# facebookresearch/CODD

Measured on AMD Instinct MI355X. Metric: frames/sec full CODD forward @960x540 (whole job), higher is better.
Workload: dtype f32 (split-bf16 MFMA operands, f32 accumulate; HITNet + context network + Fusion exact f32); 1 GPU; full CODD (HITNetMF + Motion/RAFT3D iters=16 + Fusion) 960x540 padded to 960x576, max_disp=320, one video per GPU, steady-state frames (idx>=1), synthetic stereo sequence, random-init weights; conv_precision=split, hip_graph=True, frames_per_gpu=304, prewarm_frames=150, side_streams=True, library=codd_amd/csrc/libcodd_hip.so, full=False

## Files before the change

### codd_amd/csrc/conv.hip

```cpp
#include "conv_quad_kernel.h"
#include <stdio.h>
#include <stdlib.h>

CONV_ALL_GROUPS(CONV_DECLARE)
CONVQ_ALL(CONVQ_DECLARE)
CONVQ_MULTI(CONVQM_DECLARE)


__global__ void conv_pack_kernel(const float* __restrict__ w, float* __restrict__ wp, int Cout, int Cin, int ntaps,
                                 int mb, int ck, int wrow, int nchunks, long long total, long long co_stride,
                                 long long ci_stride, float scale) {
  long long e = (long long)blockIdx.x * blockDim.x + threadIdx.x;
  if (e >= total) return;
  int col = (int)(e % wrow);
  long long t = e / wrow;
  int c = (int)(t % ck); t /= ck;
  int tap = (int)(t % ntaps); t /= ntaps;
  int chunk = (int)(t % nchunks);
  int cog = (int)(t / nchunks);
  int co = cog * 16 * mb + col, ci = chunk * ck + c;
  float v = 0.f;
  if (col < 16 * mb && co < Cout && ci < Cin) v = w[(size_t)co * co_stride + (size_t)ci * ci_stride + tap] * scale;
  wp[e] = v;
}

__global__ void conv_pack_quad_kernel(const float* __restrict__ w, float* __restrict__ wp, int Cout, int Cin, int ntaps,
                                      int mb, int ck, int nchunks, long long total) {
  long long e = (long long)blockIdx.x * blockDim.x + threadIdx.x;
  if (e >= total) return;
  const int q = (int)(e & 3);
  long long t = e >> 2;
  const int col = (int)(t % (16 * mb)); t /= 16 * mb;
  const int cq = (int)(t % (ck >> 2)); t /= ck >> 2;
  const int tap = (int)(t % ntaps); t /= ntaps;
  const int chunk = (int)(t % nchunks);
  const int cog = (int)(t / nchunks);
  const int co = cog * 16 * mb + col, ci = chunk * ck + 4 * cq + q;
  wp[e] = (co < Cout && ci < Cin) ? w[((size_t)co * Cin + ci) * ntaps + tap] : 0.f;
}

extern "C" long long codd_conv2d_packed_size_quad(int Cout, int Cin, int kh, int kw, int mb, int ck) {
  if (mb < 1 || !(ck == 16 || ck == 32)) return -1;
  return (long long)cdiv(Cout, 16 * mb) * cdiv(Cin, ck) * (kh * kw) * ck * 16 * mb;
}

extern "C" int codd_conv2d_pack_weights_quad(const float* w, float* wpacked, int Cout, int Cin, int kh, int kw, int mb,
                                             int ck, void* stream) {
  const long long total = codd_conv2d_packed_size_quad(Cout, Cin, kh, kw, mb, ck);
  if (total <= 0 || !w || !wpacked) return CODD_EINVAL;
  conv_pack_quad_kernel<<<cdiv(total, 256), 256, 0, (hipStream_t)stream>>>(w, wpacked, Cout, Cin, kh * kw, mb, ck,
                                                                           cdiv(Cin, ck), total);
  CODD_LAUNCH_CHECK();
  return CODD_OK;
}

static inline int wrow_of(int mb) { return 16 * mb + ((mb & 1) ? 0 : 16); }

extern "C" long long codd_conv2d_packed_size(int Cout, int Cin, int kh, int kw, int mb, int ck) {
  if (mb < 1 || ck < 4 || (ck & 3)) return -1;
  long long ncog = cdiv(Cout, 16 * mb), nchunks = cdiv(Cin, ck);
  return ncog * nchunks * (long long)(kh * kw) * ck * wrow_of(mb);
}

extern "C" int codd_conv2d_pack_weights_ex(const float* w, float* wpacked, int Cout, int Cin, int kh, int kw, int mb,
                                           int ck, long long co_stride, long long ci_stride, float scale,
                                           void* stream) {
  long long total = codd_conv2d_packed_size(Cout, Cin, kh, kw, mb, ck);
  if (total <= 0 || !w || !wpacked) return CODD_EINVAL;
  int nchunks = cdiv(Cin, ck);
  conv_pack_kernel<<<cdiv(total, 256), 256, 0, (hipStream_t)stream>>>(w, wpacked, Cout, Cin, kh * kw, mb, ck,
                                                                      wrow_of(mb), nchunks, total, co_stride,
                                                                      ci_stride, scale);
  CODD_LAUNCH_CHECK();
  return CODD_OK;
}

extern "C" int codd_conv2d_pack_weights(const float* w, float* wpacked, int Cout, int Cin, int kh, int kw, int mb,
                                        int ck, void* stream) {
  return codd_conv2d_pack_weights_ex(w, wpacked, Cout, Cin, kh, kw, mb, ck, (long long)Cin * kh * kw,
                                     (long long)kh * kw, 1.f, stream);
}

template <int NW, int NPB, int MB, int WREG, int IREG>
static int launch_conv(const ConvK& k, size_t lds, int grid, hipStream_t s) {
  if (lds > 64 * 1024) {
    hipError_t e = hipFuncSetAttribute((const void*)conv_mfma_kernel<NW, NPB, MB, WREG, IREG>,
                                       hipFuncAttributeMaxDynamicSharedMemorySize, (int)lds);
    if (e != hipSuccess) return (int)e;
  }
  conv_mfma_kernel<NW, NPB, MB, WREG, IREG><<<grid, NW * 64, lds, s>>>(k);
  CODD_LAUNCH_CHECK();
  return CODD_OK;
}

template <int NPB, int MB>
static int launch_conv_regs(const ConvK& k, size_t lds, int grid, hipStream_t s) {
  const int wr = cdiv(k.wchunk >> 2, 256), ir = cdiv(k.nunits, 256);
  if (wr <= 4 && ir <= 4) return launch_conv<4, NPB, MB, 4, 4>(k, lds, grid, s);
  if (wr <= 4 && ir <= 8) return launch_conv<4, NPB, MB, 4, 8>(k, lds, grid, s);
  if (wr <= 12 && ir <= 4) return launch_conv<4, NPB, MB, 12, 4>(k, lds, grid, s);
  if (wr <= 12 && ir <= 8) return launch_conv<4, NPB, MB, 12, 8>(k, lds, grid, s);
  if (wr <= 16 && ir <= 8) return launch_conv<4, NPB, MB, 16, 8>(k, lds, grid, s);
  return CODD_EUNSUPPORTED;
}

template <int NW, int MB>
static int launch_conv_nwx(const ConvK& k, size_t lds, int grid, hipStream_t s) {
  const int wr = cdiv(k.wchunk >> 2, NW * 64), ir = cdiv(k.nunits, NW * 64);
  if (wr <= 8 && ir <= 4) return launch_conv<NW, 1, MB, 8, 4>(k, lds, grid, s);
  if (wr <= 16 && ir <= 4) return launch_conv<NW, 1, MB, 16, 4>(k, lds, grid, s);
  return CODD_EUNSUPPORTED;
}

template <int NW, int NPB, int MB, int WREG, int QREG>
static int launch_quad(const ConvK& k, size_t lds, int grid, hipStream_t s) {
  if (lds > 64 * 1024) {
    hipError_t e = hipFuncSetAttribute((const void*)conv_quad_kernel<NW, NPB, MB, WREG, QREG>,
                                       hipFuncAttributeMaxDynamicSharedMemorySize, (int)lds);
    if (e != hipSuccess) return (int)e;
  }
  conv_quad_kernel<NW, NPB, MB, WREG, QREG><<<grid, NW * 64, lds, s>>>(k);
  CODD_LAUNCH_CHECK();
  return CODD_OK;
}

static int launch_quad_any(const ConvK& k, int nw, size_t lds, int grid, hipStream_t s) {
  const codd_conv_params& p = k.p;
  const int nt = nw * 64, wr = cdiv(k.wchunk >> 2, nt), qr = cdiv((p.ck >> 2) * k.upc, nt);
#define Q(W, N, M, R, QQ) if (nw == W && p.npb == N && p.mb == M && wr <= R && qr <= QQ) return launch_quad<W, N, M, R, QQ>(k, lds, grid, s);
  Q(4, 1, 1, 8, 2) Q(4, 1, 2, 8, 1) Q(4, 1, 2, 16, 2) Q(4, 1, 4, 12, 1) Q(4, 1, 4, 16, 2)
  Q(4, 2, 1, 8, 2) Q(4, 2, 2, 8, 2) Q(4, 2, 2, 16, 2) Q(4, 2, 4, 12, 2) Q(4, 2, 4, 16, 2)
  Q(4, 4, 1, 8, 4) Q(4, 4, 2, 8, 4)
  Q(9, 1, 1, 8, 1) Q(9, 1, 2, 8, 1) Q(9, 1, 4, 8, 1) Q(9, 1, 4, 16, 1)
#undef Q
  return CODD_EUNSUPPORTED;
}

int codd_conv2d_bf16(const codd_conv_params* pp, void* stream, int dry_run);

extern "C" int codd_conv2d_check(const codd_conv_params* pp) {
  if (!pp || pp->layout != 2) return CODD_EINVAL;
  return codd_conv2d_bf16(pp, nullptr, 1);
}

static int conv_fill(const codd_conv_params* pp, ConvK& k, size_t& lds, long long& grid, int& nw) {
  k.p = *pp;
  const codd_conv_params& p = k.p;
  if (!p.in0.ptr || !p.out || !p.wpacked || p.C0 <= 0 || p.C1 < 0 || (p.C1 > 0 && !p.in1.ptr)) return CODD_EINVAL;
  if (p.ck < 4 || (p.ck & 3) || p.B < 1 || p.Cout < 1 || p.kh < 1 || p.kw < 1 || p.pad_l < 0 || p.pad_t < 0)
    return CODD_EINVAL;
  if (!(p.mb == 1 || p.mb == 2 || p.mb == 4) || !(p.npb == 1 || p.npb == 2 || p.npb == 4)) return CODD_EINVAL;
  if (p.store_mode && (p.kh != 1 || p.kw != 1 || p.res1.ptr || p.res2.ptr || p.post.ptr)) return CODD_EUNSUPPORTED;
  k.cin = p.C0 + p.C1;
  k.nchunks = cdiv(k.cin, p.ck);
  k.ntaps = p.kh * p.kw;
  const int xb = p.npb >= 2 ? 2 : 1, rpw = p.npb / xb;
  nw = p.nw ? p.nw : 4;
  if (nw != 4 && (!(nw == 9 || nw == 2 || nw == 8) || p.npb != 1)) return CODD_EUNSUPPORTED;
  k.th = nw * rpw;
  k.tw = 16 * xb;
  k.thi = (k.th - 1) * p.sy + (p.kh - 1) * p.dil_y + 1;
  k.twi = (k.tw - 1) * p.sx + (p.kw - 1) * p.dil_x + 1;
  k.xoff = (4 - (p.pad_l % 4)) % 4;
  k.twp = ((k.xoff + k.twi + 3) / 4) * 4;
  k.twp4 = k.twp / 4;
  k.upc = k.thi * k.twp4;
  k.nunits = p.ck * k.upc;
  const int per = k.thi * k.twp;
  if (p.sx == 1) k.chs = ((per + 15) / 32) * 32 + 16;
  else k.chs = per + 4;
  k.wrow = wrow_of(p.mb);
  k.wchunk = k.ntaps * p.ck * k.wrow;
  k.tiles_x = cdiv(p.Wout, k.tw);
  k.tiles_y = cdiv(p.Hout, k.th);
  k.cout_eff = p.store_mode ? 4 * p.Cout : p.Cout;
  k.ncog = cdiv(k.cout_eff, 16 * p.mb);
  const size_t hwb = (size_t)p.Hin * p.Win * sizeof(float);
  k.vec_ok = (p.Win % 4 == 0) && ((uintptr_t)p.in0.ptr % 16 == 0) && (hwb % 16 == 0) &&
             (p.C1 == 0 || (uintptr_t)p.in1.ptr % 16 == 0);
  lds = ((size_t)k.wchunk + (size_t)p.ck * k.chs) * sizeof(float);
  if (p.layout == 1) {
    if (!(p.ck == 16 || p.ck == 32) || p.sx > 2 || !k.vec_ok) return CODD_EUNSUPPORTED;
    k.wchunk = k.ntaps * p.ck * 16 * p.mb;
    lds = ((size_t)k.wchunk + (size_t)p.ck * k.thi * k.twp) * sizeof(float);
  } else if (p.layout != 0) {
    return CODD_EINVAL;
  }
  if (lds > 160 * 1024) return CODD_EUNSUPPORTED;
  grid = (long long)k.tiles_x * k.tiles_y * k.ncog * p.B;
  if (grid <= 0 || grid > 0x7fffffffLL) return CODD_EINVAL;
  k.xcd = 1;
  return CODD_OK;
}

extern "C" int codd_conv2d(const codd_conv_params* pp, void* stream) {
  if (!pp) return CODD_EINVAL;
  if (pp->layout != 2 && (pp->dil2 || pp->gate)) return CODD_EUNSUPPORTED;
  if (pp->layout == 2) {
    const codd_conv_params& q = *pp;
    if (!q.xs || (!q.out && !q.xso) || !q.wpacked || q.C0 <= 0 || q.C1 < 0 || q.B < 1 || q.Cout < 1 || q.kh < 1 || q.kw < 1 ||
        q.pad_l < 0 || q.pad_t < 0)
      return CODD_EINVAL;
    if (q.store_mode && (q.kh != 1 || q.kw != 1 || q.res1.ptr || q.res2.ptr || q.post.ptr)) return CODD_EUNSUPPORTED;
    return codd_conv2d_bf16(pp, stream, 0);
  }
  ConvK k;
  size_t lds;
  long long grid;
  int nw;
  const int rc = conv_fill(pp, k, lds, grid, nw);
  if (rc != CODD_OK) return rc;
  const codd_conv_params& p = k.p;
  hipStream_t s = (hipStream_t)stream;
  if (p.layout == 1) return launch_quad_any(k, nw, lds, (int)grid, s);
#define CASEW(W, M) if (nw == W && p.mb == M) return launch_conv_nwx<W, M>(k, lds, (int)grid, s)
  CASEW(9, 1); CASEW(9, 2); CASEW(9, 4); CASEW(2, 1); CASEW(2, 2); CASEW(2, 4); CASEW(8, 1); CASEW(8, 2); CASEW(8, 4);
#undef CASEW
#define CASE(N, M) if (p.npb == N && p.mb == M) return launch_conv_regs<N, M>(k, lds, (int)grid, s)
  CASE(1, 1); CASE(1, 2); CASE(1, 4);
  CASE(2, 1); CASE(2, 2); CASE(2, 4);
  CASE(4, 1); CASE(4, 2); CASE(4, 4);
#undef CASE
  return CODD_EUNSUPPORTED;
}

template <int NW, int NPB, int MB, int WREG, int QREG>
static int launch_quad_multi(const ConvKN& kn, size_t lds, int grid, hipStream_t s) {
  if (lds > 64 * 1024) {
    hipError_t e = hipFuncSetAttribute((const void*)conv_quad_multi_kernel<NW, NPB, MB, WREG, QREG>,
                                       hipFuncAttributeMaxDynamicSharedMemorySize, (int)lds);
    if (e != hipSuccess) return (int)e;
  }
  conv_quad_multi_kernel<NW, NPB, MB, WREG, QREG><<<grid, NW * 64, lds, s>>>(kn);
  CODD_LAUNCH_CHECK();
  return CODD_OK;
}

extern "C" int codd_conv2d_multi(const codd_conv_params* ps, int n, void* stream) {
  if (!ps || n < 1 || n > CONVQ_MULTI_MAX) return CODD_EINVAL;
  if (n == 1) return codd_conv2d(ps, stream);
  ConvKN kn;
  memset(&kn, 0, sizeof(kn));
  size_t lds = 0;
  long long total = 0;
  int wr = 0, qr = 0;
  for (int i = 0; i < n; ++i) {
    size_t l;
    long long g;
    int nw;
    if (ps[i].layout != 1) return CODD_EUNSUPPORTED;
    const int rc = conv_fill(&ps[i], kn.k[i], l, g, nw);
    if (rc != CODD_OK) return rc;
    const codd_conv_params& p = kn.k[i].p;
    if (nw != 4 || p.npb != 1 || p.mb != ps[0].mb || !(p.mb == 1 || p.mb == 2)) return CODD_EUNSUPPORTED;
    const int w_ = cdiv(kn.k[i].wchunk >> 2, 256), q_ = cdiv((p.ck >> 2) * kn.k[i].upc, 256);
    wr = w_ > wr ? w_ : wr;
    qr = q_ > qr ? q_ : qr;
    lds = l > lds ? l : lds;
    kn.start[i] = (int)total;
    total += g;
  }
  for (int i = n; i <= CONVQ_MULTI_MAX; ++i) kn.start[i] = (int)total;
  if (total > 0x7fffffffLL) return CODD_EINVAL;
  hipStream_t s = (hipStream_t)stream;
  if (ps[0].mb == 1 && wr <= 8 && qr <= 2) return launch_quad_multi<4, 1, 1, 8, 2>(kn, lds, (int)total, s);
  if (ps[0].mb == 2 && wr <= 16 && qr <= 2) return launch_quad_multi<4, 1, 2, 16, 2>(kn, lds, (int)total, s);
  return CODD_EUNSUPPORTED;
}

extern "C" int codd_avgpool2(const float* in, int BC, int h, int w, float* out, void* stream);

#define CORR_MB 4
#define CORR_CK 32
extern "C" long long codd_allpairs_corr_scratch(int B, int D, int h, int w) {
  long long packed = codd_conv2d_packed_size(h * w, D, 1, 1, CORR_MB, CORR_CK);
  long long pooled = 0;
  int hh = h, ww = w;
  for (int i = 1; i < 4; ++i) { hh >>= 1; ww >>= 1; pooled += (long long)D * hh * ww; }
  return (long long)B * (packed + pooled);
}

extern "C" int codd_allpairs_corr(const float* f1, const float* f2, int B, int D, int h, int w, float* lvl0,
                                  float* lvl1, float* lvl2, float* lvl3, float* scratch, void* stream) {
  if (!f1 || !f2 || !lvl0 || !lvl1 || !lvl2 || !lvl3 || !scratch || (h >> 3) < 1 || (w >> 3) < 1) return CODD_EINVAL;
  const int N = h * w;
  const long long packed = codd_conv2d_packed_size(N, D, 1, 1, CORR_MB, CORR_CK);
  float* lv[4] = {lvl0, lvl1, lvl2, lvl3};
  for (int b = 0; b < B; ++b) {
    float* wp = scratch + (size_t)b * packed;
    int rc = codd_conv2d_pack_weights_ex(f1 + (size_t)b * D * N, wp, N, D, 1, 1, CORR_MB, CORR_CK, 1, N, 1.f / 16.f,
                                         stream);
    if (rc) return rc;
  }
  float* pool = scratch + (size_t)B * packed;
  const float* src = f2;
  int hh = h, ww = w;
  for (int i = 0; i < 4; ++i) {
    if (i > 0) {
      int rc = codd_avgpool2(src, B * D, hh, ww, pool, stream);
      if (rc) return rc;
      src = pool;
      hh >>= 1; ww >>= 1;
      pool += (size_t)B * D * hh * ww;
    }
    for (int b = 0; b < B; ++b) {
      codd_conv_params p;
      memset(&p, 0, sizeof(p));
      p.in0.ptr = src + (size_t)b * D * hh * ww; p.in0.ctot = D; p.in0.coff = 0;
      p.C0 = D; p.C1 = 0; p.B = 1; p.Hin = hh; p.Win = ww;
      p.wpacked = scratch + (size_t)b * packed;
      p.out = lv[i] + (size_t)b * N * hh * ww; p.out_ctot = N; p.out_coff = 0;
      p.Cout = N; p.Hout = hh; p.Wout = ww;
      p.kh = p.kw = 1; p.sy = p.sx = 1; p.dil_y = p.dil_x = 1;
      p.act = CODD_ACT_NONE; p.mb = CORR_MB; p.ck = CORR_CK;
      p.npb = 1;
      int rc = codd_conv2d(&p, stream);
      if (rc) return rc;
    }
  }
  return CODD_OK;
}
```

### codd_amd/csrc/conv_kernel.h

```cpp
#pragma once
#include "common.h"
#include <stdint.h>
#include <string.h>


struct ConvK {
  codd_conv_params p;
  int cin, nchunks, ntaps;
  int th, tw, thi, twi, chs;
  int wrow, wchunk;
  int tiles_x, tiles_y, ncog;
  int cout_eff;
  int twp;
  int xoff;
  int twp4;
  int upc;
  int nunits;
  int vec_ok;
  int xcd;
};

__device__ __forceinline__ int conv_xcd_item(int bid, int nwg) {
  const int q = nwg >> 3, r = nwg & 7, x = bid & 7, idx = bid >> 3;
  return (x < r ? x * (q + 1) : r * (q + 1) + (x - r) * q) + idx;
}

__device__ __forceinline__ const float* view_ptr(const codd_view& v, int b, int c, int hw) {
  return v.ptr + ((size_t)b * v.ctot + v.coff + c) * (size_t)hw;
}

template <int NPB, int MB, int DEAD>
__device__ __forceinline__ void conv_epilogue(const ConvK& k, const f32x4 (&acc)[NPB][MB], int b, int cog, int ty, int tx,
                                              int wave, int g, int j) {
  const codd_conv_params& p = k.p;
  constexpr int XB = NPB >= 2 ? 2 : 1;
  constexpr int RPW = NPB / XB;
  constexpr int NBLK = NPB * MB;
  constexpr int BLK = NBLK <= 2 ? NBLK : (DEAD >= 48 ? 4 : 2);
  static_assert(NBLK % BLK == 0, "batch");
  const int hwout = p.Hout * p.Wout;
#ifdef CONV_NO_EPILOGUE
  {
    float s_ = 0.f;
#pragma unroll
    for (int a = 0; a < NPB; ++a)
#pragma unroll
      for (int m = 0; m < MB; ++m) s_ += acc[a][m][0] + acc[a][m][1] + acc[a][m][2] + acc[a][m][3];
    const int oy = ty * k.th + wave * RPW, ox = tx * k.tw + j;
    const int co = cog * MB * 16 + 4 * g;
    if (oy < p.Hout && ox < p.Wout && co < k.cout_eff && p.store_mode == 0)
      p.out[((size_t)b * p.out_ctot + p.out_coff + co) * (size_t)hwout + oy * p.Wout + ox] = s_;
    return;
  }
#endif
  bool cok[MB][4], pok[NPB], anyp = false;
  int oy[NPB], ox[NPB];
#pragma unroll
  for (int m = 0; m < MB; ++m)
#pragma unroll
    for (int r = 0; r < 4; ++r) cok[m][r] = (cog * MB + m) * 16 + 4 * g + r < k.cout_eff;
#pragma unroll
  for (int a = 0; a < NPB; ++a) {
    oy[a] = ty * k.th + wave * RPW + a / XB;
    ox[a] = tx * k.tw + (a % XB) * 16 + j;
    pok[a] = oy[a] < p.Hout && ox[a] < p.Wout;
    anyp |= pok[a];
  }
  if (p.store_mode == 0) {
    int pix[NPB];
#pragma unroll
    for (int a = 0; a < NPB; ++a) pix[a] = oy[a] * p.Wout + ox[a];
#pragma unroll
    for (int q0 = 0; q0 < NBLK; q0 += BLK) {
      float bv[BLK][4], r1[BLK][4], r2[BLK][4], po[BLK][4];
#define CONV_EPI_LOAD(DST, VIEW)                                                         \
  _Pragma("unroll") for (int i = 0; i < BLK; ++i)                                        \
  _Pragma("unroll") for (int r = 0; r < 4; ++r) {                                        \
    const int a = (q0 + i) % NPB, m = (q0 + i) / NPB;                                    \
    DST[i][r] = 0.f;                                                                     \
    if (VIEW.ptr && pok[a] && cok[m][r])                                                 \
      DST[i][r] = view_ptr(VIEW, b, (cog * MB + m) * 16 + 4 * g + r, hwout)[pix[a]];     \
  }
#pragma unroll
      for (int i = 0; i < BLK; ++i)
#pragma unroll
        for (int r = 0; r < 4; ++r) {
          const int a = (q0 + i) % NPB, m = (q0 + i) / NPB;
          bv[i][r] = 0.f;
          if (p.bias && pok[a] && cok[m][r]) bv[i][r] = p.bias[(cog * MB + m) * 16 + 4 * g + r];
        }
      CONV_EPI_LOAD(r1, p.res1)
      CONV_EPI_LOAD(r2, p.res2)
      CONV_EPI_LOAD(po, p.post)
#undef CONV_EPI_LOAD
      float v[BLK][4];
#pragma unroll
      for (int i = 0; i < BLK; ++i)
#pragma unroll
        for (int r = 0; r < 4; ++r) {
          const int a = (q0 + i) % NPB, m = (q0 + i) / NPB;
          float t = acc[a][m][r];
          if (p.bias) t += bv[i][r];
          if (p.res1.ptr) t += r1[i][r];
          if (p.res2.ptr) t += r2[i][r];
          t = act_apply(t, p.act, (cog * MB + m) * 16 + 4 * g + r);
          if (p.post.ptr) t += po[i][r];
          v[i][r] = t;
        }
#pragma unroll
      for (int i = 0; i < BLK; ++i)
#pragma unroll
        for (int r = 0; r < 4; ++r) {
          const int a = (q0 + i) % NPB, m = (q0 + i) / NPB;
          if (pok[a] && cok[m][r])
            p.out[((size_t)b * p.out_ctot + p.out_coff + (cog * MB + m) * 16 + 4 * g + r) * (size_t)hwout + pix[a]] = v[i][r];
        }
    }
  } else {
    const int W2 = 2 * p.Wout;
#pragma unroll
    for (int m = 0; m < MB; ++m) {
      int cq[4], cc[4];
      float bv[4];
#pragma unroll
      for (int r = 0; r < 4; ++r) {
        const int co = (cog * MB + m) * 16 + 4 * g + r;
        cq[r] = co / p.Cout;
        cc[r] = co - cq[r] * p.Cout;
        bv[r] = 0.f;
        if (p.bias && anyp && cok[m][r]) bv[r] = p.bias[cc[r]];
      }
#pragma unroll
      for (int a = 0; a < NPB; ++a)
#pragma unroll
        for (int r = 0; r < 4; ++r) {
          if (!pok[a] || !cok[m][r]) continue;
          float t = acc[a][m][r];
          if (p.bias) t += bv[r];
          t = act_apply(t, p.act, cc[r]);
          p.out[((size_t)b * p.out_ctot + p.out_coff + cc[r]) * (size_t)(4 * hwout) +
                (size_t)(2 * oy[a] + (cq[r] >> 1)) * W2 + 2 * ox[a] + (cq[r] & 1)] = t;
        }
    }
  }
}

template <int NW, int NPB, int MB, int WREG, int IREG>
__global__ __launch_bounds__(NW * 64) void conv_mfma_kernel(const ConvK k) {
  constexpr int NT = NW * 64;
  extern __shared__ __attribute__((aligned(16))) float smem[];
  float* wl = smem;
  float* il = smem + k.wchunk;
  const codd_conv_params& p = k.p;
  const int tid = threadIdx.x, lane = tid & 63, wave = tid >> 6;
  const int g = lane >> 4, j = lane & 15;
  constexpr int XB = NPB >= 2 ? 2 : 1;
  constexpr int RPW = NPB / XB;

  int bid = k.xcd ? conv_xcd_item(blockIdx.x, gridDim.x) : blockIdx.x;
  const int tx = bid % k.tiles_x; bid /= k.tiles_x;
  const int ty = bid % k.tiles_y; bid /= k.tiles_y;
  const int cog = bid % k.ncog;
  const int b = bid / k.ncog;

  const int hwin = p.Hin * p.Win;
  const int gy0 = ty * k.th * p.sy - p.pad_t;
  const int gxs = tx * k.tw * p.sx - p.pad_l - k.xoff;

  int u_lds[IREG], u_g[IREG], u_c[IREG];
  unsigned u_m[IREG];
#pragma unroll
  for (int r = 0; r < IREG; ++r) {
    const int u = tid + r * NT;
    u_c[r] = -1; u_m[r] = 0; u_lds[r] = 0; u_g[r] = 0;
    if (u < k.nunits) {
      const int c = u / k.upc, rem = u - c * k.upc;
      const int y = rem / k.twp4, x4 = rem - y * k.twp4;
      const int gy = gy0 + y, gx = gxs + 4 * x4;
      unsigned m = 0;
      if ((unsigned)gy < (unsigned)p.Hin) {
#pragma unroll
        for (int q = 0; q < 4; ++q) m |= ((unsigned)(gx + q) < (unsigned)p.Win) ? (1u << q) : 0u;
      }
      u_c[r] = c; u_m[r] = m;
      u_lds[r] = c * k.chs + y * k.twp + 4 * x4;
      u_g[r] = gy * p.Win + gx;
    }
  }
  const int wchunk4 = k.wchunk >> 2;
  float4 wreg[WREG], ireg[IREG];

#define CONV_ISSUE(CH)                                                                                    \
  {                                                                                                       \
    const float4* src_ = (const float4*)(p.wpacked + ((size_t)(cog * k.nchunks + (CH))) * k.wchunk);      \
    _Pragma("unroll") for (int r = 0; r < WREG; ++r) {                                                    \
      const int e = tid + r * NT;                                                                         \
      wreg[r] = e < wchunk4 ? src_[e] : make_float4(0.f, 0.f, 0.f, 0.f);                                  \
    }                                                                                                     \
    const int c0_ = (CH) * p.ck;                                                                          \
    _Pragma("unroll") for (int r = 0; r < IREG; ++r) {                                                    \
      float4 v = make_float4(0.f, 0.f, 0.f, 0.f);                                                         \
      const int cg = c0_ + u_c[r];                                                                        \
      if (u_c[r] >= 0 && cg < k.cin && u_m[r]) {                                                          \
        const float* s_ =                                                                                 \
            (cg < p.C0 ? view_ptr(p.in0, b, cg, hwin) : view_ptr(p.in1, b, cg - p.C0, hwin)) + u_g[r];    \
        if (u_m[r] == 0xFu && k.vec_ok) {                                                                 \
          v = *(const float4*)s_;                                                                         \
        } else {                                                                                          \
          if (u_m[r] & 1u) v.x = s_[0];                                                                   \
          if (u_m[r] & 2u) v.y = s_[1];                                                                   \
          if (u_m[r] & 4u) v.z = s_[2];                                                                   \
          if (u_m[r] & 8u) v.w = s_[3];                                                                   \
        }                                                                                                 \
      }                                                                                                   \
      ireg[r] = v;                                                                                        \
    }                                                                                                     \
  }
#define CONV_COMMIT()                                                                                     \
  {                                                                                                       \
    float4* dst_ = (float4*)wl;                                                                           \
    _Pragma("unroll") for (int r = 0; r < WREG; ++r) {                                                    \
      const int e = tid + r * NT;                                                                         \
      if (e < wchunk4) dst_[e] = wreg[r];                                                                 \
    }                                                                                                     \
    _Pragma("unroll") for (int r = 0; r < IREG; ++r) if (u_c[r] >= 0) *(float4*)(il + u_lds[r]) = ireg[r]; \
  }

  f32x4 acc[NPB][MB];
#pragma unroll
  for (int a = 0; a < NPB; ++a)
#pragma unroll
    for (int m = 0; m < MB; ++m) acc[a][m] = (f32x4){0.f, 0.f, 0.f, 0.f};

  int pbase[NPB];
#pragma unroll
  for (int a = 0; a < NPB; ++a) {
    const int prow = wave * RPW + a / XB, pcol = (a % XB) * 16 + j;
    pbase[a] = prow * p.sy * k.twp + pcol * p.sx + k.xoff;
  }

  CONV_ISSUE(0);
  for (int ch = 0; ch < k.nchunks; ++ch) {
    __syncthreads();
    CONV_COMMIT();
    __syncthreads();
    if (ch + 1 < k.nchunks) CONV_ISSUE(ch + 1);
    for (int ky = 0; ky < p.kh; ++ky) {
      for (int kx = 0; kx < p.kw; ++kx) {
        const float* wp = wl + (ky * p.kw + kx) * p.ck * k.wrow + j + g * k.wrow;
        const float* ip = il + ky * p.dil_y * k.twp + kx * p.dil_x + g * k.chs;
        const int wstep = 4 * k.wrow, istep = 4 * k.chs;
#pragma unroll 4
        for (int c4 = 0; c4 < p.ck; c4 += 4) {
          float av[MB], bv[NPB];
#pragma unroll
          for (int m = 0; m < MB; ++m) av[m] = wp[m * 16];
#pragma unroll
          for (int a = 0; a < NPB; ++a) bv[a] = ip[pbase[a]];
          wp += wstep;
          ip += istep;
#pragma unroll
          for (int a = 0; a < NPB; ++a)
#pragma unroll
            for (int m = 0; m < MB; ++m)
              acc[a][m] = __builtin_amdgcn_mfma_f32_16x16x4f32(av[m], bv[a], acc[a][m], 0, 0, 0);
        }
      }
    }
  }

  conv_epilogue<NPB, MB, 4 * WREG + 4 * IREG>(k, acc, b, cog, ty, tx, wave, g, j);
}

#define CONV_REGS_NW4(X, NPB, MB) X(4, NPB, MB, 4, 4) X(4, NPB, MB, 4, 8) X(4, NPB, MB, 12, 4) X(4, NPB, MB, 12, 8) X(4, NPB, MB, 16, 8)
#define CONV_REGS_NWX(X, NW, MB) X(NW, 1, MB, 8, 4) X(NW, 1, MB, 16, 4)
#define CONV_GROUP_0(X) CONV_REGS_NW4(X, 1, 1)
#define CONV_GROUP_1(X) CONV_REGS_NW4(X, 1, 2)
#define CONV_GROUP_2(X) CONV_REGS_NW4(X, 1, 4)
#define CONV_GROUP_3(X) CONV_REGS_NW4(X, 2, 1) CONV_REGS_NW4(X, 2, 2)
#define CONV_GROUP_4(X) CONV_REGS_NW4(X, 2, 4) CONV_REGS_NW4(X, 4, 1)
#define CONV_GROUP_5(X) CONV_REGS_NW4(X, 4, 2)
#define CONV_GROUP_6(X) CONV_REGS_NW4(X, 4, 4)
#define CONV_GROUP_7(X) CONV_REGS_NWX(X, 9, 1) CONV_REGS_NWX(X, 9, 2) CONV_REGS_NWX(X, 9, 4)
#define CONV_GROUP_8(X) CONV_REGS_NWX(X, 2, 1) CONV_REGS_NWX(X, 2, 2) CONV_REGS_NWX(X, 2, 4)
#define CONV_GROUP_9(X) CONV_REGS_NWX(X, 8, 1) CONV_REGS_NWX(X, 8, 2) CONV_REGS_NWX(X, 8, 4)
#define CONV_ALL_GROUPS(X) CONV_GROUP_0(X) CONV_GROUP_1(X) CONV_GROUP_2(X) CONV_GROUP_3(X) CONV_GROUP_4(X) CONV_GROUP_5(X) CONV_GROUP_6(X) CONV_GROUP_7(X) CONV_GROUP_8(X) CONV_GROUP_9(X)
#define CONV_DECLARE(NW, NPB, MB, WREG, IREG) extern template __global__ void conv_mfma_kernel<NW, NPB, MB, WREG, IREG>(const ConvK);
#define CONV_DEFINE(NW, NPB, MB, WREG, IREG) template __global__ void conv_mfma_kernel<NW, NPB, MB, WREG, IREG>(const ConvK);
```

### codd_amd/csrc/conv_quad_kernel.h

```cpp
#pragma once
#include "conv_kernel.h"

template <int NW, int NPB, int MB, int WREG, int QREG>
__device__ __forceinline__ void conv_quad_body(const ConvK& k, int bid, float* smem) {
  constexpr int NT = NW * 64;
  float* wl = smem;
  float* il = smem + k.wchunk;
  const codd_conv_params& p = k.p;
  const int tid = threadIdx.x, lane = tid & 63, wave = tid >> 6;
  const int g = lane >> 4, j = lane & 15;
  constexpr int XB = NPB >= 2 ? 2 : 1;
  constexpr int RPW = NPB / XB;

  const int tx = bid % k.tiles_x; bid /= k.tiles_x;
  const int ty = bid % k.tiles_y; bid /= k.tiles_y;
  const int cog = bid % k.ncog;
  const int b = bid / k.ncog;

  const int hwin = p.Hin * p.Win;
  const int gy0 = ty * k.th * p.sy - p.pad_t;
  const int gxs = tx * k.tw * p.sx - p.pad_l - k.xoff;

  const int ncq = p.ck >> 2;
  const int nq = ncq * k.upc;
  int q_lds[QREG], q_g[QREG], q_c[QREG];
  bool q_in[QREG];
#pragma unroll
  for (int r = 0; r < QREG; ++r) {
    const int u = tid + r * NT;
    q_c[r] = -1; q_in[r] = false; q_lds[r] = 0; q_g[r] = 0;
    if (u < nq) {
      const int cq = u / k.upc, rem = u - cq * k.upc;
      const int y = rem / k.twp4, x4 = rem - y * k.twp4;
      const int gy = gy0 + y, gx = gxs + 4 * x4;
      q_c[r] = 4 * cq;
      q_in[r] = (unsigned)gy < (unsigned)p.Hin && gx >= 0 && gx + 3 < p.Win;
      q_lds[r] = ((cq * k.thi + y) * k.twp + 4 * x4) * 4;
      q_g[r] = gy * p.Win + gx;
    }
  }
  const int wchunk4 = k.wchunk >> 2;
  float4 wreg[WREG], ireg[QREG][4];

#define QUAD_ISSUE(CH)                                                                                    \
  {                                                                                                       \
    const float4* src_ = (const float4*)(p.wpacked + ((size_t)(cog * k.nchunks + (CH))) * k.wchunk);      \
    _Pragma("unroll") for (int r = 0; r < WREG; ++r) {                                                    \
      const int e = tid + r * NT;                                                                         \
      wreg[r] = e < wchunk4 ? src_[e] : make_float4(0.f, 0.f, 0.f, 0.f);                                  \
    }                                                                                                     \
    _Pragma("unroll") for (int r = 0; r < QREG; ++r) {                                                    \
      _Pragma("unroll") for (int c = 0; c < 4; ++c) {                                                     \
        float4 v = make_float4(0.f, 0.f, 0.f, 0.f);                                                       \
        const int cg = (CH) * p.ck + q_c[r] + c;                                                          \
        if (q_c[r] >= 0 && q_in[r] && cg < k.cin) {                                                       \
          const float* s_ =                                                                               \
              (cg < p.C0 ? view_ptr(p.in0, b, cg, hwin) : view_ptr(p.in1, b, cg - p.C0, hwin)) + q_g[r];  \
          v = *(const float4*)s_;                                                                         \
        }                                                                                                 \
        ireg[r][c] = v;                                                                                   \
      }                                                                                                   \
    }                                                                                                     \
  }
#define QUAD_COMMIT()                                                                                     \
  {                                                                                                       \
    float4* dst_ = (float4*)wl;                                                                           \
    _Pragma("unroll") for (int r = 0; r < WREG; ++r) {                                                    \
      const int e = tid + r * NT;                                                                         \
      if (e < wchunk4) dst_[e] = wreg[r];                                                                 \
    }                                                                                                     \
    _Pragma("unroll") for (int r = 0; r < QREG; ++r) if (q_c[r] >= 0) {                                   \
      float4* d_ = (float4*)(il + q_lds[r]);   \
      d_[0] = make_float4(ireg[r][0].x, ireg[r][1].x, ireg[r][2].x, ireg[r][3].x);                        \
      d_[1] = make_float4(ireg[r][0].y, ireg[r][1].y, ireg[r][2].y, ireg[r][3].y);                        \
      d_[2] = make_float4(ireg[r][0].z, ireg[r][1].z, ireg[r][2].z, ireg[r][3].z);                        \
      d_[3] = make_float4(ireg[r][0].w, ireg[r][1].w, ireg[r][2].w, ireg[r][3].w);                        \
    }                                                                                                     \
  }

  f32x4 acc[NPB][MB];
#pragma unroll
  for (int a = 0; a < NPB; ++a)
#pragma unroll
    for (int m = 0; m < MB; ++m) acc[a][m] = (f32x4){0.f, 0.f, 0.f, 0.f};

  int pbase[NPB];
#pragma unroll
  for (int a = 0; a < NPB; ++a) {
    const int prow = wave * RPW + a / XB, pcol = (a % XB) * 16 + j;
    pbase[a] = prow * p.sy * k.twp + pcol * p.sx + k.xoff;
  }
  const int wq = 16 * MB;
  const int iq = k.thi * k.twp;
  const int ngr = p.ck >> 4;

  QUAD_ISSUE(0);
  for (int ch = 0; ch < k.nchunks; ++ch) {
    __syncthreads();
    QUAD_COMMIT();
    __syncthreads();
    if (ch + 1 < k.nchunks) QUAD_ISSUE(ch + 1);
    const float4* w4 = (const float4*)wl;
    const float4* i4 = (const float4*)il;
    for (int ky = 0; ky < p.kh; ++ky) {
      for (int kx = 0; kx < p.kw; ++kx) {
        const float4* wp = w4 + ((size_t)(ky * p.kw + kx) * (p.ck >> 2) + g) * wq + j;
        const float4* ip = i4 + (size_t)g * iq + ky * p.dil_y * k.twp + kx * p.dil_x;
        for (int gr = 0; gr < ngr; ++gr) {
          float4 av[MB], bv[NPB];
#pragma unroll
          for (int m = 0; m < MB; ++m) av[m] = wp[m * 16];
#pragma unroll
          for (int a = 0; a < NPB; ++a) bv[a] = ip[pbase[a]];
          wp += 4 * wq;
          ip += 4 * iq;
#pragma unroll
          for (int a = 0; a < NPB; ++a)
#pragma unroll
            for (int m = 0; m < MB; ++m) {
              acc[a][m] = __builtin_amdgcn_mfma_f32_16x16x4f32(av[m].x, bv[a].x, acc[a][m], 0, 0, 0);
              acc[a][m] = __builtin_amdgcn_mfma_f32_16x16x4f32(av[m].y, bv[a].y, acc[a][m], 0, 0, 0);
              acc[a][m] = __builtin_amdgcn_mfma_f32_16x16x4f32(av[m].z, bv[a].z, acc[a][m], 0, 0, 0);
              acc[a][m] = __builtin_amdgcn_mfma_f32_16x16x4f32(av[m].w, bv[a].w, acc[a][m], 0, 0, 0);
            }
        }
      }
    }
  }
#undef QUAD_ISSUE
#undef QUAD_COMMIT

  conv_epilogue<NPB, MB, 4 * WREG + 16 * QREG>(k, acc, b, cog, ty, tx, wave, g, j);
}

template <int NW, int NPB, int MB, int WREG, int QREG>
__global__ __launch_bounds__(NW * 64) void conv_quad_kernel(const ConvK k) {
  extern __shared__ __attribute__((aligned(16))) float smem[];
  conv_quad_body<NW, NPB, MB, WREG, QREG>(k, k.xcd ? conv_xcd_item(blockIdx.x, gridDim.x) : blockIdx.x, smem);
}

constexpr int CONVQ_MULTI_MAX = 4;
struct ConvKN {
  ConvK k[CONVQ_MULTI_MAX];
  int start[CONVQ_MULTI_MAX + 1];
};
template <int NW, int NPB, int MB, int WREG, int QREG>
__global__ __launch_bounds__(NW * 64) void conv_quad_multi_kernel(const ConvKN kn) {
  extern __shared__ __attribute__((aligned(16))) float smem[];
  const int bid = blockIdx.x;
  if (bid < kn.start[1]) conv_quad_body<NW, NPB, MB, WREG, QREG>(kn.k[0], bid, smem);
  else if (bid < kn.start[2]) conv_quad_body<NW, NPB, MB, WREG, QREG>(kn.k[1], bid - kn.start[1], smem);
  else if (bid < kn.start[3]) conv_quad_body<NW, NPB, MB, WREG, QREG>(kn.k[2], bid - kn.start[2], smem);
  else conv_quad_body<NW, NPB, MB, WREG, QREG>(kn.k[3], bid - kn.start[3], smem);
}

#define CONVQ_GROUP_A(X) X(4, 1, 2, 8, 1) X(4, 1, 2, 16, 2) X(4, 1, 4, 12, 1) X(4, 1, 4, 16, 2) X(4, 1, 1, 8, 2)
#define CONVQ_GROUP_B(X) X(4, 2, 2, 8, 2) X(4, 2, 2, 16, 2) X(4, 2, 4, 12, 2) X(4, 2, 4, 16, 2) X(4, 2, 1, 8, 2)
#define CONVQ_GROUP_C(X) X(9, 1, 2, 8, 1) X(9, 1, 4, 8, 1) X(9, 1, 4, 16, 1) X(9, 1, 1, 8, 1) X(4, 4, 1, 8, 4) X(4, 4, 2, 8, 4)
#define CONVQ_ALL(X) CONVQ_GROUP_A(X) CONVQ_GROUP_B(X) CONVQ_GROUP_C(X)
#define CONVQ_DECLARE(NW, NPB, MB, WREG, QREG) extern template __global__ void conv_quad_kernel<NW, NPB, MB, WREG, QREG>(const ConvK);
#define CONVQ_DEFINE(NW, NPB, MB, WREG, QREG) template __global__ void conv_quad_kernel<NW, NPB, MB, WREG, QREG>(const ConvK);
#define CONVQ_MULTI(X) X(4, 1, 1, 8, 2) X(4, 1, 2, 16, 2)
#define CONVQM_DECLARE(NW, NPB, MB, WREG, QREG) extern template __global__ void conv_quad_multi_kernel<NW, NPB, MB, WREG, QREG>(const ConvKN);
#define CONVQM_DEFINE(NW, NPB, MB, WREG, QREG) template __global__ void conv_quad_multi_kernel<NW, NPB, MB, WREG, QREG>(const ConvKN);
```

Before: 105.1 frames/s.

## Transpose MFMA operands so conv epilogue stores contiguous pixels as float4

Swaps the A/B operands of the f32 MFMA in the direct and quad conv kernels, so each lane's four accumulator values now cover four consecutive output pixels of one channel instead of four channels of one pixel. The epilogue is rewritten for this layout: a single bias load per channel, 16-byte vectorized residual/post loads and output stores when the pointers are aligned, and an activation switch hoisted out of the per-element loop. It also adds a min-blocks launch bound for one variant and adjusts the epilogue batching threshold. The aim is to cut scattered scalar global stores in the epilogue. The risk is that the unaligned fallback path, the pixel-shuffle store path and register pressure change with the new layout.

```diff
diff --git a/codd_amd/csrc/conv.hip b/codd_amd/csrc/conv.hip
--- a/codd_amd/csrc/conv.hip
+++ b/codd_amd/csrc/conv.hip
@@ -178,6 +178,8 @@
   const size_t hwb = (size_t)p.Hin * p.Win * sizeof(float);
   k.vec_ok = (p.Win % 4 == 0) && ((uintptr_t)p.in0.ptr % 16 == 0) && (hwb % 16 == 0) &&
              (p.C1 == 0 || (uintptr_t)p.in1.ptr % 16 == 0);
+  const auto al16 = [](const void* q) { return (uintptr_t)q % 16 == 0; };
+  k.evec = p.store_mode == 0 && p.Wout % 4 == 0 && al16(p.out) && al16(p.res1.ptr) && al16(p.res2.ptr) && al16(p.post.ptr);
   lds = ((size_t)k.wchunk + (size_t)p.ck * k.chs) * sizeof(float);
   if (p.layout == 1) {
     if (!(p.ck == 16 || p.ck == 32) || p.sx > 2 || !k.vec_ok) return CODD_EUNSUPPORTED;
diff --git a/codd_amd/csrc/conv_kernel.h b/codd_amd/csrc/conv_kernel.h
--- a/codd_amd/csrc/conv_kernel.h
+++ b/codd_amd/csrc/conv_kernel.h
@@ -17,6 +17,7 @@
   int upc;
   int nunits;
   int vec_ok;
+  int evec;
   int xcd;
 };
 
@@ -29,14 +30,59 @@
   return v.ptr + ((size_t)b * v.ctot + v.coff + c) * (size_t)hw;
 }
 
+template <int N>
+__device__ __forceinline__ void conv_epi_act(float (&v)[N][4], const float (&po)[N][4], bool post, int act,
+                                             const int (&co)[N]) {
+#pragma clang fp contract(off)
+#define CONV_EPI_ARM(ACT)                                                 \
+  case ACT:                                                               \
+    _Pragma("unroll") for (int i = 0; i < N; ++i)                         \
+    _Pragma("unroll") for (int r = 0; r < 4; ++r) {                       \
+      float t = act_apply(v[i][r], ACT, co[i]);                           \
+      if (post) t += po[i][r];                                            \
+      v[i][r] = t;                                                        \
+    }                                                                     \
+    break;
+  switch (act) {
+    CONV_EPI_ARM(CODD_ACT_LRELU02)
+    CONV_EPI_ARM(CODD_ACT_RELU)
+    CONV_EPI_ARM(CODD_ACT_SIGMOID)
+    CONV_EPI_ARM(CODD_ACT_TANH)
+    CONV_EPI_ARM(CODD_ACT_MISH)
+    CONV_EPI_ARM(CODD_ACT_RELU_CH0)
+    default:
+#pragma unroll
+      for (int i = 0; i < N; ++i)
+#pragma unroll
+        for (int r = 0; r < 4; ++r)
+          if (post) v[i][r] += po[i][r];
+  }
+#undef CONV_EPI_ARM
+}
+
+template <int N>
+__device__ __forceinline__ void conv_epi_act(float (&v)[N][4], int act, int co) {
+  float none[N][4];
+  int cos[N];
+#pragma unroll
+  for (int i = 0; i < N; ++i) {
+    cos[i] = co;
+#pragma unroll
+    for (int r = 0; r < 4; ++r) none[i][r] = 0.f;
+  }
+  conv_epi_act<N>(v, none, false, act, cos);
+}
+
 template <int NPB, int MB, int DEAD>
-__device__ __forceinline__ void conv_epilogue(const ConvK& k, const f32x4 (&acc)[NPB][MB], int b, int cog, int ty, int tx,
-                                              int wave, int g, int j) {
+__device__ __forceinline__ void conv_epilogue(const ConvK& k, const f32x4 (&acc)[NPB][MB], int b, int cog, int ty, int tx) {
   const codd_conv_params& p = k.p;
+  int t_ = threadIdx.x;
+  asm volatile("" : "+v"(t_));
+  const int wave = t_ >> 6, g = (t_ & 63) >> 4, j = t_ & 15;
   constexpr int XB = NPB >= 2 ? 2 : 1;
   constexpr int RPW = NPB / XB;
   constexpr int NBLK = NPB * MB;
-  constexpr int BLK = NBLK <= 2 ? NBLK : (DEAD >= 48 ? 4 : 2);
+  constexpr int BLK = NBLK <= 2 ? NBLK : (DEAD >= 52 ? 4 : 2);
   static_assert(NBLK % BLK == 0, "batch");
   const int hwout = p.Hout * p.Wout;
 #ifdef CONV_NO_EPILOGUE
@@ -46,25 +92,27 @@
     for (int a = 0; a < NPB; ++a)
 #pragma unroll
       for (int m = 0; m < MB; ++m) s_ += acc[a][m][0] + acc[a][m][1] + acc[a][m][2] + acc[a][m][3];
-    const int oy = ty * k.th + wave * RPW, ox = tx * k.tw + j;
-    const int co = cog * MB * 16 + 4 * g;
+    const int oy = ty * k.th + wave * RPW, ox = tx * k.tw + 4 * g;
+    const int co = cog * MB * 16 + j;
     if (oy < p.Hout && ox < p.Wout && co < k.cout_eff && p.store_mode == 0)
       p.out[((size_t)b * p.out_ctot + p.out_coff + co) * (size_t)hwout + oy * p.Wout + ox] = s_;
     return;
   }
 #endif
-  bool cok[MB][4], pok[NPB], anyp = false;
+  bool cok[MB];
+  unsigned pm[NPB];
   int oy[NPB], ox[NPB];
 #pragma unroll
-  for (int m = 0; m < MB; ++m)
-#pragma unroll
-    for (int r = 0; r < 4; ++r) cok[m][r] = (cog * MB + m) * 16 + 4 * g + r < k.cout_eff;
+  for (int m = 0; m < MB; ++m) cok[m] = (cog * MB + m) * 16 + j < k.cout_eff;
 #pragma unroll
   for (int a = 0; a < NPB; ++a) {
     oy[a] = ty * k.th + wave * RPW + a / XB;
-    ox[a] = tx * k.tw + (a % XB) * 16 + j;
-    pok[a] = oy[a] < p.Hout && ox[a] < p.Wout;
-    anyp |= pok[a];
+    ox[a] = tx * k.tw + (a % XB) * 16 + 4 * g;
+    pm[a] = 0;
+    if (oy[a] < p.Hout) {
+#pragma unroll
+      for (int r = 0; r < 4; ++r) pm[a] |= (ox[a] + r < p.Wout) ? (1u << r) : 0u;
+    }
   }
   if (p.store_mode == 0) {
     int pix[NPB];
@@ -72,26 +120,41 @@
     for (int a = 0; a < NPB; ++a) pix[a] = oy[a] * p.Wout + ox[a];
 #pragma unroll
     for (int q0 = 0; q0 < NBLK; q0 += BLK) {
-      float bv[BLK][4], r1[BLK][4], r2[BLK][4], po[BLK][4];
-#define CONV_EPI_LOAD(DST, VIEW)                                                         \
-  _Pragma("unroll") for (int i = 0; i < BLK; ++i)                                        \
-  _Pragma("unroll") for (int r = 0; r < 4; ++r) {                                        \
-    const int a = (q0 + i) % NPB, m = (q0 + i) / NPB;                                    \
-    DST[i][r] = 0.f;                                                                     \
-    if (VIEW.ptr && pok[a] && cok[m][r])                                                 \
-      DST[i][r] = view_ptr(VIEW, b, (cog * MB + m) * 16 + 4 * g + r, hwout)[pix[a]];     \
-  }
-#pragma unroll
-      for (int i = 0; i < BLK; ++i)
-#pragma unroll
-        for (int r = 0; r < 4; ++r) {
-          const int a = (q0 + i) % NPB, m = (q0 + i) / NPB;
-          bv[i][r] = 0.f;
-          if (p.bias && pok[a] && cok[m][r]) bv[i][r] = p.bias[(cog * MB + m) * 16 + 4 * g + r];
-        }
-      CONV_EPI_LOAD(r1, p.res1)
-      CONV_EPI_LOAD(r2, p.res2)
-      CONV_EPI_LOAD(po, p.post)
+      float bv[BLK], r1[BLK][4], r2[BLK][4], po[BLK][4];
+      int co[BLK];
+      bool ok[BLK];
+#pragma unroll
+      for (int i = 0; i < BLK; ++i) {
+        const int a = (q0 + i) % NPB, m = (q0 + i) / NPB;
+        co[i] = (cog * MB + m) * 16 + j;
+        ok[i] = cok[m] && pm[a] != 0;
+        bv[i] = 0.f;
+        if (p.bias && ok[i]) bv[i] = p.bias[co[i]];
+      }
+#define CONV_EPI_LOAD(DST, VIEW, VEC)                                                    \
+  _Pragma("unroll") for (int i = 0; i < BLK; ++i) {                                      \
+    const int a = (q0 + i) % NPB;                                                        \
+    _Pragma("unroll") for (int r = 0; r < 4; ++r) DST[i][r] = 0.f;                       \
+    if (VIEW.ptr && ok[i]) {                                                             \
+      const float* s_ = view_ptr(VIEW, b, co[i], hwout) + pix[a];                        \
+      if (VEC) {                                                                         \
+        const f32x4 q_ = *(const f32x4*)s_;                                              \
+        DST[i][0] = q_[0]; DST[i][1] = q_[1]; DST[i][2] = q_[2]; DST[i][3] = q_[3];      \
+      } else {                                                                           \
+        _Pragma("unroll") for (int r = 0; r < 4; ++r)                                    \
+          if (pm[a] & (1u << r)) DST[i][r] = s_[r];                                      \
+      }                                                                                  \
+    }                                                                                    \
+  }
+      if (k.evec) {
+        CONV_EPI_LOAD(r1, p.res1, true)
+        CONV_EPI_LOAD(r2, p.res2, true)
+        CONV_EPI_LOAD(po, p.post, true)
+      } else {
+        CONV_EPI_LOAD(r1, p.res1, false)
+        CONV_EPI_LOAD(r2, p.res2, false)
+        CONV_EPI_LOAD(po, p.post, false)
+      }
 #undef CONV_EPI_LOAD
       float v[BLK][4];
 #pragma unroll
@@ -100,53 +163,64 @@
         for (int r = 0; r < 4; ++r) {
           const int a = (q0 + i) % NPB, m = (q0 + i) / NPB;
           float t = acc[a][m][r];
-          if (p.bias) t += bv[i][r];
+          if (p.bias) t += bv[i];
           if (p.res1.ptr) t += r1[i][r];
           if (p.res2.ptr) t += r2[i][r];
-          t = act_apply(t, p.act, (cog * MB + m) * 16 + 4 * g + r);
-          if (p.post.ptr) t += po[i][r];
           v[i][r] = t;
         }
-#pragma unroll
-      for (int i = 0; i < BLK; ++i)
-#pragma unroll
-        for (int r = 0; r < 4; ++r) {
-          const int a = (q0 + i) % NPB, m = (q0 + i) / NPB;
-          if (pok[a] && cok[m][r])
-            p.out[((size_t)b * p.out_ctot + p.out_coff + (cog * MB + m) * 16 + 4 * g + r) * (size_t)hwout + pix[a]] = v[i][r];
+      conv_epi_act<BLK>(v, po, p.post.ptr != nullptr, p.act, co);
+#pragma unroll
+      for (int i = 0; i < BLK; ++i) {
+        const int a = (q0 + i) % NPB;
+        if (!ok[i]) continue;
+        float* d_ = p.out + ((size_t)b * p.out_ctot + p.out_coff + co[i]) * (size_t)hwout + pix[a];
+        if (k.evec) {
+          *(f32x4*)d_ = (f32x4){v[i][0], v[i][1], v[i][2], v[i][3]};
+        } else {
+#pragma unroll
+          for (int r = 0; r < 4; ++r)
+            if (pm[a] & (1u << r)) d_[r] = v[i][r];
         }
+      }
     }
   } else {
     const int W2 = 2 * p.Wout;
+    bool anyp = false;
+#pragma unroll
+    for (int a = 0; a < NPB; ++a) anyp |= pm[a] != 0;
 #pragma unroll
     for (int m = 0; m < MB; ++m) {
-      int cq[4], cc[4];
-      float bv[4];
-#pragma unroll
-      for (int r = 0; r < 4; ++r) {
-        const int co = (cog * MB + m) * 16 + 4 * g + r;
-        cq[r] = co / p.Cout;
-        cc[r] = co - cq[r] * p.Cout;
-        bv[r] = 0.f;
-        if (p.bias && anyp && cok[m][r]) bv[r] = p.bias[cc[r]];
-      }
+      const int co = (cog * MB + m) * 16 + j;
+      const int cq = co / p.Cout, cc = co - cq * p.Cout;
+      float bv = 0.f;
+      if (p.bias && anyp && cok[m]) bv = p.bias[cc];
+      float v[NPB][4];
 #pragma unroll
       for (int a = 0; a < NPB; ++a)
 #pragma unroll
         for (int r = 0; r < 4; ++r) {
-          if (!pok[a] || !cok[m][r]) continue;
           float t = acc[a][m][r];
-          if (p.bias) t += bv[r];
-          t = act_apply(t, p.act, cc[r]);
-          p.out[((size_t)b * p.out_ctot + p.out_coff + cc[r]) * (size_t)(4 * hwout) +
-                (size_t)(2 * oy[a] + (cq[r] >> 1)) * W2 + 2 * ox[a] + (cq[r] & 1)] = t;
+          if (p.bias) t += bv;
+          v[a][r] = t;
         }
-    }
-  }
+      conv_epi_act<NPB>(v, p.act, cc);
+      if (!cok[m]) continue;
+      float* d_ = p.out + ((size_t)b * p.out_ctot + p.out_coff + cc) * (size_t)(4 * hwout) + (size_t)(cq >> 1) * W2 + (cq & 1);
+#pragma unroll
+      for (int a = 0; a < NPB; ++a)
+#pragma unroll
+        for (int r = 0; r < 4; ++r)
+          if (pm[a] & (1u << r)) d_[(size_t)(2 * oy[a]) * W2 + 2 * (ox[a] + r)] = v[a][r];
+    }
+  }
+}
+
+constexpr int conv_min_blocks(int nw, int npb, int mb, int wreg, int ireg) {
+  return (nw == 4 && npb == 2 && mb == 2 && wreg == 4 && ireg == 8) ? 4 : 0;
 }
 
 template <int NW, int NPB, int MB, int WREG, int IREG>
-__global__ __launch_bounds__(NW * 64) void conv_mfma_kernel(const ConvK k) {
+__global__ __launch_bounds__(NW * 64, conv_min_blocks(NW, NPB, MB, WREG, IREG)) void conv_mfma_kernel(const ConvK k) {
   constexpr int NT = NW * 64;
   extern __shared__ __attribute__((aligned(16))) float smem[];
   float* wl = smem;
@@ -263,13 +337,13 @@
           for (int a = 0; a < NPB; ++a)
 #pragma unroll
             for (int m = 0; m < MB; ++m)
-              acc[a][m] = __builtin_amdgcn_mfma_f32_16x16x4f32(av[m], bv[a], acc[a][m], 0, 0, 0);
+              acc[a][m] = __builtin_amdgcn_mfma_f32_16x16x4f32(bv[a], av[m], acc[a][m], 0, 0, 0);
         }
       }
     }
   }
 
-  conv_epilogue<NPB, MB, 4 * WREG + 4 * IREG>(k, acc, b, cog, ty, tx, wave, g, j);
+  conv_epilogue<NPB, MB, 4 * WREG + 4 * IREG>(k, acc, b, cog, ty, tx);
 }
 
 #define CONV_REGS_NW4(X, NPB, MB) X(4, NPB, MB, 4, 4) X(4, NPB, MB, 4, 8) X(4, NPB, MB, 12, 4) X(4, NPB, MB, 12, 8) X(4, NPB, MB, 16, 8)
diff --git a/codd_amd/csrc/conv_quad_kernel.h b/codd_amd/csrc/conv_quad_kernel.h
--- a/codd_amd/csrc/conv_quad_kernel.h
+++ b/codd_amd/csrc/conv_quad_kernel.h
@@ -118,10 +118,10 @@
           for (int a = 0; a < NPB; ++a)
 #pragma unroll
             for (int m = 0; m < MB; ++m) {
-              acc[a][m] = __builtin_amdgcn_mfma_f32_16x16x4f32(av[m].x, bv[a].x, acc[a][m], 0, 0, 0);
-              acc[a][m] = __builtin_amdgcn_mfma_f32_16x16x4f32(av[m].y, bv[a].y, acc[a][m], 0, 0, 0);
-              acc[a][m] = __builtin_amdgcn_mfma_f32_16x16x4f32(av[m].z, bv[a].z, acc[a][m], 0, 0, 0);
-              acc[a][m] = __builtin_amdgcn_mfma_f32_16x16x4f32(av[m].w, bv[a].w, acc[a][m], 0, 0, 0);
+              acc[a][m] = __builtin_amdgcn_mfma_f32_16x16x4f32(bv[a].x, av[m].x, acc[a][m], 0, 0, 0);
+              acc[a][m] = __builtin_amdgcn_mfma_f32_16x16x4f32(bv[a].y, av[m].y, acc[a][m], 0, 0, 0);
+              acc[a][m] = __builtin_amdgcn_mfma_f32_16x16x4f32(bv[a].z, av[m].z, acc[a][m], 0, 0, 0);
+              acc[a][m] = __builtin_amdgcn_mfma_f32_16x16x4f32(bv[a].w, av[m].w, acc[a][m], 0, 0, 0);
             }
         }
       }
@@ -130,7 +130,7 @@
 #undef QUAD_ISSUE
 #undef QUAD_COMMIT
 
-  conv_epilogue<NPB, MB, 4 * WREG + 16 * QREG>(k, acc, b, cog, ty, tx, wave, g, j);
+  conv_epilogue<NPB, MB, 4 * WREG + 16 * QREG>(k, acc, b, cog, ty, tx);
 }
 
 template <int NW, int NPB, int MB, int WREG, int QREG>
```

Result: faster. 106.8 frames/s (median of 6 runs) (+1.6%).
